# jolars/sgdnet

Measured on AMD Instinct MI355X. Metric: saga_epochs_per_sec, higher is better.
Workload: dtype f64

## Files before the change

sgdnet_amd/csrc/batched_k1.hpp:

```cpp
#pragma once

#include "batched_device.hpp"
#include "r_rng_word.hpp"

namespace sgdnet {


constexpr int kLanes8 = 8;

struct RecHeader {
  double y;
  int nnz;
  int ovf;
};

template <int kThreads>
__device__ __forceinline__ double k1_lanes8_draws(const SagaDev& d, const uint32_t* sp, int lo, int hi, double b0,
                                                  const double* wv, double* Dl) {
  typedef int ipair_t __attribute__((ext_vector_type(2)));
  typedef double dpair_t __attribute__((ext_vector_type(2)));
  constexpr int U = 4;
  constexpr int kG = kThreads / kLanes8;
  constexpr int kStep = kG * U;
  const int gl = threadIdx.x & (kLanes8 - 1);
// ... 65 lines not shown
          if (nz > kInReg8) {
            const int ov = __shfl(hd.ovf, 2 * u, kLanes8);
            row_for_each<kInReg8, kLanes8>(d, d.rec + (size_t)su[u] * stride, nz, ov, gl,
                      [&](int64_t j, double v) { scatter_add<true>(Dl + j, v * gc); });
          }
        }
      }
    }
    gct += gcp;
  }
  return gct;
}

constexpr int kCQ = 12;
constexpr int kCYOff = 112;
constexpr uint32_t kLongBit = 0x80000000u;
constexpr uint32_t kYBit = 0x20000000u;
constexpr int kCMOff = 120;

template <class F>
__device__ __forceinline__ void row_tail_compact(const SagaDev& d, uint32_t sid, int nnz, int gl, int E, F f) {
  const char* qb = d.cQ + (size_t)sid * kCStride;
  for (int e = E + 4 + gl; e < nnz; e += kLanes8) {
    if (e < E + kCQ) {
      f((int64_t) reinterpret_cast<const uint16_t*>(qb + 8)[e - E],
        reinterpret_cast<const double*>(qb + 32)[e - E]);
    } else {
      const int64_t q0 = d.ptr[sid];
      f((int64_t)d.idx[q0 + e], d.val[q0 + e]);
    }
  }
}

constexpr int kTicket = 32;

struct TicketSource {
  int* counter;
  int lo, hi, m;
  int t = 0;
  bool dynamic;
  __device__ __forceinline__ int next() {
    if (!dynamic) {
      const int b = lo + (t++ * (kLdsBlock / 64) + (int)(threadIdx.x >> 6)) * kTicket;
      return b < hi ? b : m;
    }
    int b = 0;
    if ((threadIdx.x & 63) == 0)
      b = __hip_atomic_fetch_add(counter, kTicket, __ATOMIC_RELAXED, __HIP_MEMORY_SCOPE_WORKGROUP);
    b = lo + __builtin_amdgcn_readfirstlane(b);
    return b < hi ? b : m;
  }
};

template <bool kRawStream>
struct K1CompactT {
  typedef double dpair_t __attribute__((ext_vector_type(2)));
  static constexpr int U = 4;
  int E, in_reg, gl, g, q, slot, id_off, v_off;
  bool y_in_meta, is_owner, in_p, half;
  const char* plane;
  char* P;
  const uint32_t* sp;
  const uint32_t* meta;
  int m;
  TicketSource tk;
  int b_cur, b_nxt;
  uint32_t s_cur, s_nxt;
  bool raw = false;
  const double* par = nullptr;

  __device__ __forceinline__ uint32_t sample_id(uint32_t x) const {
    if (kRawStream && raw) x = (uint32_t)par[1] + word_to_draw(x, par[0]);
    return x;
  }

  __device__ __forceinline__ int own_pos(int base) const { return base + U * g + q < m ? base + U * g + q : base; }
  __device__ __forceinline__ uint32_t tagged(uint32_t sid) const {
    const uint32_t mb = (meta[sid >> 4] >> (2 * (sid & 15))) & 3u;
    return sid | ((mb & 1u) ? kLongBit : 0u) | ((mb & 2u) ? kYBit : 0u);
  }
  static __device__ __forceinline__ int static_tickets() { return 2 * (kLdsBlock / 64) * kTicket; }

  __device__ __forceinline__ void init(const SagaDev& d, const uint32_t* sp_, int m_, int blk, int nblk,
                                       int* ticket_counter) {
    E = d.cE;
    in_reg = E + 4;
    y_in_meta = E == 12;
    gl = threadIdx.x & (kLanes8 - 1);
    g = (threadIdx.x & 63) >> 3;
    q = gl >> 1;
    is_owner = (gl & 1) == 0;
    in_p = gl < 6;
    slot = in_p ? gl : gl - 6;
    P = d.cP;
    plane = in_p ? d.cP : d.cQ;
    id_off = in_p ? 8 * E + 4 * slot : 8 + 4 * slot;
    v_off = in_p ? 16 * slot : 32 + 16 * slot;
    half = in_p && slot == 5 && E == 11;
    sp = sp_;
    meta = d.cmeta;
    m = m_;
    const int share = ((m + nblk - 1) / nblk + kTicket - 1) / kTicket * kTicket;
    tk.counter = ticket_counter;
    tk.lo = blk * share;
    tk.hi = tk.lo + share < m ? tk.lo + share : m;
    tk.m = m;
    tk.dynamic = share >= 4 * (kLdsBlock / 64) * kTicket;
    tk.t = 2;
    const int wave = (int)(threadIdx.x >> 6);
    b_cur = tk.lo + wave * kTicket;
    b_nxt = tk.lo + ((kLdsBlock / 64) + wave) * kTicket;
    if (b_cur >= tk.hi) b_cur = m;
    if (b_nxt >= tk.hi) b_nxt = m;
  }
  __device__ __forceinline__ void request_first() {
    s_cur = b_cur < m ? sp[own_pos(b_cur)] : 0u;
    s_nxt = b_nxt < m ? sp[own_pos(b_nxt)] : 0u;
  }
  __device__ __forceinline__ void begin(const SagaDev& d, const uint32_t* sp_, int m_, int blk, int nblk,
                                        int* ticket_counter) {
    init(d, sp_, m_, blk, nblk, ticket_counter);
    request_first();
  }

  __device__ __forceinline__ void tag_first() {
    if (b_cur < m) s_cur = tagged(sample_id(s_cur));
  }

  __device__ __forceinline__ double run(const SagaDev& d, double b0, const double* wv, double* Dl) {
    double gct = 0.0;
    while (b_cur < m) {
      const bool v_own = b_cur + U * g + q < m;
      uint32_t su[U];
#pragma unroll
      for (int u = 0; u < U; ++u) su[u] = (uint32_t)__shfl((int)s_cur, 2 * u, kLanes8);
      const uint32_t s_this = s_cur & kIdMask;
      double y_own = (s_cur & kYBit) ? 1.0 : 0.0;
      if (!y_in_meta) y_own = *reinterpret_cast<const double*>(P + (size_t)s_this * kCStride + kCYOff);
      int nnz_own = 0;
      if (s_cur & kLongBit) nnz_own = *reinterpret_cast<const int*>(d.cQ + (size_t)s_this * kCStride);
      uint32_t jf[U];
      dpair_t vf[U];
#pragma unroll
      for (int u = 0; u < U; ++u) {
        const bool on = in_p || (su[u] & kLongBit) != 0;
        const char* base = plane + (size_t)(su[u] & kIdMask) * kCStride;
        jf[u] = 0u;
        vf[u] = dpair_t{0.0, 0.0};
        if (on) {
          jf[u] = *reinterpret_cast<const uint32_t*>(base + id_off);
          vf[u] = *reinterpret_cast<const dpair_t*>(base + v_off);
        }
      }
      const int b_nn = b_nxt < m ? tk.next() : m;
      uint32_t s_nn = 0u;
      if (b_nn < m) s_nn = sp[own_pos(b_nn)];
      if (b_nxt < m) s_nxt = tagged(sample_id(s_nxt));
      if (half) {
#pragma unroll
        for (int u = 0; u < U; ++u) {
          vf[u].y = 0.0;
          jf[u] &= 0xffffu;
        }
      }
      double acc[U];
#pragma unroll
      for (int u = 0; u < U; ++u) acc[u] = vf[u].x * wv[jf[u] & 0xffffu] + vf[u].y * wv[jf[u] >> 16];
      const bool own_tail = v_own && nnz_own > in_reg;
      const bool any_tail = __ballot(own_tail) != 0;
      if (any_tail) {
#pragma unroll
        for (int u = 0; u < U; ++u) {
          const int nz = __shfl(own_tail ? nnz_own : 0, 2 * u, kLanes8);
          if (nz > in_reg) {
            double a = 0.0;
            row_tail_compact(d, su[u] & kIdMask, nz, gl, E, [&](int64_t j, double v) { a += v * wv[j]; });
            acc[u] += a;
          }
        }
      }
      const bool hi4 = (gl & 4) != 0, hi2 = (gl & 2) != 0;
      const double r0 = (hi4 ? acc[2] : acc[0]) + __shfl_xor(hi4 ? acc[0] : acc[2], 4, kLanes8);
      const double r1 = (hi4 ? acc[3] : acc[1]) + __shfl_xor(hi4 ? acc[1] : acc[3], 4, kLanes8);
      double t = (hi2 ? r1 : r0) + __shfl_xor(hi2 ? r0 : r1, 2, kLanes8);
      t += __shfl_xor(t, 1, kLanes8);
      const double lp = t + b0;
      const double g0 = d.family == SGDNET_BINOMIAL ? 1.0 - y_own - 1.0 / (1.0 + exp(lp)) : lp - y_own;
      double gcp = 0.0;
      if (is_owner && v_own) {
        const double old = __hip_atomic_exchange(reinterpret_cast<double*>(P + (size_t)s_this * kCStride + kCMOff), g0,
                                                 __ATOMIC_RELAXED, __HIP_MEMORY_SCOPE_AGENT);
        gcp = g0 - old;
      }
#pragma unroll
      for (int u = 0; u < U; ++u) {
        const double gc = __shfl(gcp, 2 * u, kLanes8);
        if (gc != 0.0) {
          if (vf[u].x != 0.0) scatter_add<true>(Dl + (jf[u] & 0xffffu), vf[u].x * gc);
          if (vf[u].y != 0.0) scatter_add<true>(Dl + (jf[u] >> 16), vf[u].y * gc);
          if (any_tail) {
            const int nz = __shfl(own_tail ? nnz_own : 0, 2 * u, kLanes8);
            if (nz > in_reg)
              row_tail_compact(d, su[u] & kIdMask, nz, gl, E,
                               [&](int64_t j, double v) { scatter_add<true>(Dl + j, v * gc); });
          }
        }
      }
      gct += gcp;
      s_cur = s_nxt;
      s_nxt = s_nn;
      b_cur = b_nxt;
      b_nxt = b_nn;
    }
    return gct;
  }
};
typedef K1CompactT<false> K1Compact;

template <int U>
struct K1IdsOnly {
  uint32_t s[U];
  bool valid[U];
  uint32_t s_own;
  bool v_own;
  bool valid_any;
  __device__ __forceinline__ void load(const SagaDev& d, const uint32_t* sp, int i, int hi, int step, int gl,
                                       int safe) {
#pragma unroll
    for (int u = 0; u < U; ++u) {
      const int iu = i + u * step;
      valid[u] = iu < hi;
      s[u] = sp[valid[u] ? iu : safe];
    }
    const int q = U == 4 ? gl >> 2 : gl;
    const int iq = i + q * step;
    v_own = q < U && iq < hi;
    s_own = sp[v_own ? iq : safe];
  }
};

template <int U>
struct K1Draws {
  uint32_t s[U];
  int jf[U], nnz[U];
  double vf[U];
  double gcp;
  bool valid[U];
  uint32_t s_own;
  double y_own;
  bool v_own;
  static __device__ __forceinline__ int draw_of(int gl) { return U == 4 ? gl >> 2 : gl; }

  static __device__ __forceinline__ int owner(int u) { return U == 4 ? 4 * u : u; }
  static __device__ __forceinline__ bool is_owner(int gl) { return U == 4 ? (gl & 3) == 0 : gl < U; }

  __device__ __forceinline__ void load_ids(const SagaDev& d, const uint32_t* sp, int i, int hi, int step, int gl,
// ... 112 lines not shown
```

sgdnet_amd/csrc/batched_shards.hip:

```cpp
#include "batched_k1.hpp"
#include "r_rng_bodies.hpp"

namespace sgdnet {

template <int KMAX>
__global__ __launch_bounds__(kBlock) void saga_vs_sweep_kernel(SagaDev d, LamParams* lamp, int tail, int nfb) {
  __shared__ double part[kSlabGroups][kSlabElems];
  __shared__ double red[kBlock / 64];
  __shared__ double sh_d0[KMAX];
  const SweepParams q = load_sweep_params(d, lamp, tail, SweepOverride{0.0, 0.0, 0.0});
  const int K = KMAX == 1 ? 1 : d.K;
  const int F = kSlabElems / K;
  const int E = F * K;
  const int v = (int)blockIdx.x / nfb, fb = (int)blockIdx.x - v * nfb;
  const int64_t KP = (int64_t)K * d.p;
  const double n_d = d.v_size[v];
  const int e = threadIdx.x % kSlabElems, g = threadIdx.x / kSlabElems;
  const int64_t elem = (int64_t)fb * E + e;
  const int64_t j_own = (int64_t)fb * F + threadIdx.x;
  const bool updates = (int)threadIdx.x < F && j_own < d.p;
  double w_old[KMAX], g_old[KMAX], c_own = 0.0;
#pragma unroll
  for (int k = 0; k < KMAX; ++k) {
    w_old[k] = g_old[k] = 0.0;
// ... 199 lines not shown
        return false;
      }
    }
  }
}

__device__ __forceinline__ bool fused_start(unsigned* sync, LamParams* lamp, unsigned grid) {
  unsigned* go = sync + kSyncGo * kSyncLine;
  const long long t0 = wall_clock64();
  if (blockIdx.x == 0) {
    unsigned expect = 0u;
    for (;;) {
      if (sync_load(sync, kSyncStart) >= grid) {
        __hip_atomic_compare_exchange_strong(go, &expect, 1u, __ATOMIC_RELAXED, __ATOMIC_RELAXED, __HIP_MEMORY_SCOPE_AGENT);
        break;
      }
      if (sync_load(sync, kSyncGo) != 0u) break;
      if (wall_clock64() - t0 > kFusedStartTicks) {
        __hip_atomic_compare_exchange_strong(go, &expect, 2u, __ATOMIC_RELAXED, __ATOMIC_RELAXED, __HIP_MEMORY_SCOPE_AGENT);
        break;
      }
      __builtin_amdgcn_s_sleep(4);
    }
  } else {
    for (;;) {
      if (sync_load(sync, kSyncGo) != 0u) break;
      if (wall_clock64() - t0 > 2 * kFusedStartTicks) {
        unsigned expect = 0u;
        __hip_atomic_compare_exchange_strong(go, &expect, 2u, __ATOMIC_RELAXED, __ATOMIC_RELAXED, __HIP_MEMORY_SCOPE_AGENT);
        break;
      }
      __builtin_amdgcn_s_sleep(4);
    }
  }
  const unsigned decision = sync_load(sync, kSyncGo);
  if (decision != 1u && decision != 3u) {
    __hip_atomic_store(&lamp->fused_abort, 1, __ATOMIC_RELAXED, __HIP_MEMORY_SCOPE_AGENT);
    __hip_atomic_fetch_max(sync + kSyncSticky * kSyncLine, 1u, __ATOMIC_RELAXED, __HIP_MEMORY_SCOPE_AGENT);
  }
  return decision == 1u;
}

__device__ __forceinline__ double fused_block_sum(double a, double* red) {
  a = wave_sum(a);
  if ((threadIdx.x & 63) == 0) red[threadIdx.x >> 6] = a;
  __syncthreads();
  double t = 0.0;
#pragma unroll
  for (int wv = 0; wv < kLdsBlock / 64; ++wv) t += red[wv];
  __syncthreads();
  return t;
}

__device__ __forceinline__ void fused_leave(const SagaDev& d, LamParams* lamp, int nb, bool epoch_done) {
  asm volatile("s_waitcnt vmcnt(0)" ::: "memory");
  __syncthreads();
  if (threadIdx.x == 0) {
    unsigned* sync = d.vsync;
    if (epoch_done && blockIdx.x == 0) {
      end_epoch(lamp, nb);
      if (d.n_peers > 1) __hip_atomic_fetch_add(sync + kSyncSeq * kSyncLine, 1u, __ATOMIC_RELAXED, __HIP_MEMORY_SCOPE_AGENT);
    }
    const unsigned prev = __hip_atomic_fetch_add(sync + kSyncExit * kSyncLine, 1u, __ATOMIC_RELAXED, __HIP_MEMORY_SCOPE_AGENT);
    if (prev + 1u == gridDim.x) {
      for (int wd = 0; wd < kSyncLines; ++wd)
        __hip_atomic_store(sync + wd * kSyncLine, 0u, __ATOMIC_RELAXED, __HIP_MEMORY_SCOPE_AGENT);
      if (!(d.n_peers > 1))
        for (int wd = 0; wd < kFusedMaxBps; ++wd)
          __hip_atomic_store(d.vcol + wd * kSyncLine, 0u, __ATOMIC_RELAXED, __HIP_MEMORY_SCOPE_AGENT);
      if (d.rngdev && lamp->rng_generate) d.rngdev->gen += 1u;
    }
  }
}

template <bool kPeers>
__global__ __launch_bounds__(kLdsBlock) void saga_vs_epoch_kernel(SagaDev d, LamParams* lamp, int nb, int every) {
  extern __shared__ __attribute__((aligned(16))) double Dl[];
  __shared__ int ticket_counter;
  __shared__ int sh_ok;
  __shared__ double sh_red[kLdsBlock / 64];
  __shared__ double sh_val[4];
  const int tid = threadIdx.x;
  const int64_t p = d.p;
  const int64_t P2 = p >> 1;
  const int S = d.v_bps, V = d.V;
  if ((int)blockIdx.x >= V * S) {
    if (d.rngdev && lamp->rng_generate) {
      const RngDev* R = d.rngdev;
      const unsigned gen = R->gen;
      uint32_t* lds = reinterpret_cast<uint32_t*>(Dl);
      const int rb = (int)blockIdx.x - V * S, nrb = (int)gridDim.x - V * S;
      mt_state_body(rb, nrb, reinterpret_cast<uint32_t(*)[2][kMtN + 1]>(lds), R->state[gen & 1u], R->ends,
                    R->stream + (int64_t)(gen & 1u) * R->n, R->n, R->seg, R->gens);
      __syncthreads();
      mt_jump_body(rb, nrb, lds, R->state[gen & 1u], R->state[(gen + 1u) & 1u], R->poly, R->gens);
    }
    fused_leave(d, lamp, nb, false);
    return;
  }
  const int v = (int)blockIdx.x % V, wi = (int)blockIdx.x / V;
  const int F = 2 * (int)((p + 2 * S - 1) / (2 * S));
  const int j0 = wi * F;
  const int jn = p - j0 < F ? (p - j0 > 0 ? (int)(p - j0) : 0) : F;
  double* Wl = Dl + p;
  f64x2_t* D2 = reinterpret_cast<f64x2_t*>(Dl);
  f64x2_t* W2 = reinterpret_cast<f64x2_t*>(Wl);
  const int penalty = lamp->penalty;
  __shared__ double sh_par[10];
  if (tid == 0) {
    sh_par[0] = lamp->gamma;
    sh_par[1] = lamp->beta;
    sh_par[2] = lamp->r_full;
    sh_par[3] = lamp->ls_full;
    sh_par[4] = lamp->r_tail;
    sh_par[5] = lamp->ls_tail;
    double tot = 0.0, lo = 0.0;
    for (int u = 0; u < d.V; ++u) {
      tot += d.v_size[u];
      if (u < (int)blockIdx.x % d.V) lo += d.v_size[u];
    }
    sh_par[6] = d.v_size[(int)blockIdx.x % d.V];
    sh_par[7] = lo;
    sh_par[8] = tot;
  }
  const int64_t m_full = lamp->m_full;
  const int64_t sbase = lamp->stream_base;
  const bool raw_words = lamp->stream_raw != 0;
  const int64_t dps = d.v_dps;
  const bool std_x = d.standardize != 0;
  const int64_t L = 2 * p + 2;
  double* vwv = d.vw + (int64_t)v * p;
  double* vGv = d.vG + (int64_t)v * p;
  double* refv = d.vx + (int64_t)v * L;
  double* cwp = d.vx + (int64_t)V * L;
  unsigned* sync = d.vsync;
  const __amdgpu_buffer_rsrc_t rs_slab = fused_rsrc(d.slab, (int64_t)V * S * p * 8);
  const __amdgpu_buffer_rsrc_t rs_w = fused_rsrc(vwv, p * 8);
  const uint32_t* const stream_v = d.stream + sbase + (int64_t)v * dps;
  typedef K1CompactT<true> K1Epoch;
  const double* const draw_par = sh_par + 6;

#ifdef SGDNET_PHASE_TIMING
  unsigned long long ph_t = 0;
  if (d.dbg && tid == 0) d.dbg[(size_t)blockIdx.x * 16 + 14] = ph_t = phase_stamp();
#define FPH(slot)                                                 \
  do {                                                            \
    if (d.dbg && tid == 0) {                                      \
      const unsigned long long now = phase_stamp();               \
      d.dbg[(size_t)blockIdx.x * 16 + (slot)] += now - ph_t;      \
      d.dbg[(size_t)blockIdx.x * 16 + 15] = ph_t = now;           \
    }                                                             \
  } while (0)
#else
#define FPH(slot) ((void)0)
#endif
  if (tid == 0) {
    const unsigned xcc = __builtin_amdgcn_s_getreg((3 << 11) | 20) & 15u;
    __hip_atomic_fetch_or(sync + (kSyncXcd + v) * kSyncLine, 1u << xcc, __ATOMIC_RELAXED, __HIP_MEMORY_SCOPE_AGENT);
    asm volatile("s_waitcnt vmcnt(0)" ::: "memory");
    __hip_atomic_fetch_add(sync + kSyncStart * kSyncLine, 1u, __ATOMIC_RELAXED, __HIP_MEMORY_SCOPE_AGENT);
    sh_ok = fused_start(sync, lamp, (unsigned)(V * S)) ? 1 : 0;
    if (sh_ok) {
      const unsigned mask = sync_load(sync, kSyncXcd + v);
      sh_ok = (mask & (mask - 1u)) == 0u ? 3 : 1;
    }
  }
  for (int64_t i = tid; i < P2; i += kLdsBlock) D2[i] = f64x2_t{0.0, 0.0};
  __syncthreads();
  bool done = false;
  bool alive = sh_ok != 0;
  unsigned col_base = 0u;
  if (kPeers) {
    int merges = 0;
    for (int r = 0; r < nb; ++r) merges += (r + 1 == nb || (r + 1) % every == 0) ? 1 : 0;
    col_base = sync_load(sync, kSyncSeq) * (unsigned)merges;
  }
  const bool local = (sh_ok & 2) != 0 && d.vs_xcd_local != 0;
  int mi = 0;
  uint32_t s_first = 0u, s_second = 0u;
  if (alive) {
    const int m0 = (int)(dps < m_full ? dps : m_full);
    K1Epoch nx;
    nx.begin(d, stream_v, m0, wi, S, &ticket_counter);
    s_first = nx.s_cur;
    s_second = nx.s_nxt;
  }
  for (int r = 0; alive && r < nb; ++r) {
    const int64_t t0 = (int64_t)r * m_full;
    const int m = (int)(dps - t0 < m_full ? dps - t0 : m_full);
    const bool tail = m != m_full;
    const bool last = r + 1 == nb;
    const bool merge_due = last || (r + 1) % every == 0;

    if (tid == 0) ticket_counter = K1Epoch::static_tickets();
    K1Epoch cg;
    cg.init(d, stream_v + t0, m, wi, S, &ticket_counter);
    cg.raw = raw_words;
    cg.par = draw_par;
    cg.s_cur = s_first;
    cg.s_nxt = s_second;
    cg.tag_first();
    int ts = threadIdx.x;
    asm volatile("" : "+v"(ts));
    double cw = 0.0, bv = 0.0;
    if ((ts >> 6) == 0) {
      if (std_x && r > 0)
        for (int k = ts & 63; k < S; k += 64) cw += ld_sc1(cwp + v * kFusedMaxBps + k);
      bv = r == 0 ? d.b[0] : ld_sc1(d.vb + v);
    }
    {
      constexpr int kStage = 8;
      for (int64_t i0 = ts; i0 < P2; i0 += (int64_t)kLdsBlock * kStage) {
        f64x2_t t[kStage];
#pragma unroll
        for (int q = 0; q < kStage; ++q) {
          const int64_t i = i0 + (int64_t)q * kLdsBlock;
          t[q] = f64x2_t{0.0, 0.0};
          if (i < P2) t[q] = r == 0 ? reinterpret_cast<const f64x2_t*>(d.w)[i] : ld2_sc1(rs_w, (uint32_t)(i * 16));
        }
#pragma unroll
        for (int q = 0; q < kStage; ++q) {
          const int64_t i = i0 + (int64_t)q * kLdsBlock;
          if (i < P2) W2[i] = t[q];
        }
      }
    }
    if ((ts >> 6) == 0) {
      cw = wave_sum(cw);
      if ((ts & 63) == 0) sh_val[0] = bv - cw;
    }
    __syncthreads();
    if (r == 0 && std_x) {
      double a = 0.0;
      for (int64_t j = ts; j < p; j += kLdsBlock) a += d.c[j] * Wl[j];
      a = fused_block_sum(a, sh_red);
      if (ts == 0) sh_val[0] -= a;
      __syncthreads();
    }
    const double b0 = sh_val[0];
    FPH(0);

    const double gct = cg.run(d, b0, Wl, Dl);
    __syncthreads();
    FPH(1);
    int tq = threadIdx.x;
    asm volatile("" : "+v"(tq));
    const int lane = tq & 63, wave = tq >> 6;
    const int64_t t0n = t0 + m_full;
    const int mn = (int)(dps - t0n < m_full ? dps - t0n : m_full);

    {
      const uint32_t base = (uint32_t)(((int64_t)blockIdx.x * p) * 8);
      for (int64_t i = tq; i < P2; i += kLdsBlock) {
        st2_shard(D2[i], rs_slab, base + (uint32_t)(i * 16), local);
        D2[i] = f64x2_t{0.0, 0.0};
      }
      const double t = wave_sum(gct);
      if (lane == 0) sh_red[wave] = t;
      __syncthreads();
      if (tq == 0) {
        double tot = 0.0;
        for (int wv = 0; wv < kLdsBlock / 64; ++wv) tot += sh_red[wv];
        st_shard(d.vd0 + blockIdx.x, tot, local);
      }
    }
    fused_arrive(sync, kSyncCnt1 + v);
    FPH(2);
    const bool upd = tq < jn;
    const bool icpt = wi == 0 && tq == jn;
    const bool act = upd || icpt;
    const int64_t j = j0 + tq;
    const int64_t oa = upd ? j : 2 * p, ob = upd ? p + j : 2 * p + 1;
    double* const rep_a = upd ? vGv + j : d.vgb + v;
    double* const rep_b = upd ? vwv + j : d.vb + v;
    const double* const own_a = upd ? d.G + j : d.gb;
    const double* const own_b = upd ? d.w + j : d.b;
    double a_old = 0.0, b_old = 0.0, c_own = 0.0, ra = 0.0, rb = 0.0;
    if (act) {
      a_old = r == 0 ? *own_a : ld_sc1(rep_a);
      b_old = r == 0 ? *own_b : ld_sc1(rep_b);
      if (std_x && upd) c_own = d.c[j];
      if (merge_due) {
        ra = mi == 0 ? *own_a : ld_sc1(refv + oa);
        rb = mi == 0 ? *own_b : ld_sc1(refv + ob);
      }
    }
    if (tq == 0) sh_ok = fused_poll(sync, kSyncCnt1 + v, (unsigned)S * (unsigned)(r + 1), lamp) ? 1 : 0;
    __syncthreads();
    if (!sh_ok) break;
    FPH(3);

    {
      double gsum = 0.0;
      if (wave == kLdsBlock / 64 - 1)
        for (int k = lane; k < S; k += 64) gsum += ld_sc1(d.vd0 + k * V + v);
      f64x2_t acc[kFusedChunks];
#pragma unroll
      for (int c = 0; c < kFusedChunks; ++c) acc[c] = f64x2_t{0.0, 0.0};
      for (int k = wave; k < S; k += 2 * (kLdsBlock / 64)) {
        const bool two = k + kLdsBlock / 64 < S;
        const uint32_t o0 = (uint32_t)((((int64_t)(k * V + v)) * p + j0) * 8);
        const uint32_t o1 = (uint32_t)((((int64_t)((k + kLdsBlock / 64) * V + v)) * p + j0) * 8);
        f64x2_t a0[kFusedChunks], a1[kFusedChunks];
#pragma unroll
        for (int c = 0; c < kFusedChunks; ++c) {
          const int pi = c * 64 + lane;
          a0[c] = a1[c] = f64x2_t{0.0, 0.0};
          if (2 * pi < jn) {
            a0[c] = ld2_sc1(rs_slab, o0 + (uint32_t)(pi * 16));
            if (two) a1[c] = ld2_sc1(rs_slab, o1 + (uint32_t)(pi * 16));
          }
        }
#pragma unroll
        for (int c = 0; c < kFusedChunks; ++c) {
          acc[c] += a0[c];
          acc[c] += a1[c];
        }
      }
#pragma unroll
      for (int c = 0; c < kFusedChunks; ++c) {
        const int pi = c * 64 + lane;
        if (2 * pi < F) reinterpret_cast<f64x2_t*>(Wl + (int64_t)wave * F)[pi] = acc[c];
      }
      if (wave == kLdsBlock / 64 - 1) {
        gsum = wave_sum(gsum);
        if (lane == 0) sh_val[1] = gsum;
      }
    }
    __syncthreads();
    double a_new = a_old, b_new = b_old;
    {
      const double d0 = sh_val[1];
      const double n_d = sh_par[6], gamma = sh_par[0];
      if (upd) {
        double dj = 0.0;
#pragma unroll
        for (int wv = 0; wv < kLdsBlock / 64; ++wv) dj += Wl[(int64_t)wv * F + tq];
        if (std_x) dj -= c_own * d0;
        const double beta = sh_par[1];
        const double r_m = tail ? sh_par[4] : sh_par[2], ls_m = tail ? sh_par[5] : sh_par[3];
        const double val = r_m * b_old - (gamma * ls_m) * a_old - gamma * dj;
        const double tau = beta * gamma * ls_m;
        b_new = val;
        if (penalty == SGDNET_ELASTICNET) {
          b_new = soft_threshold(val, tau);
        } else if (penalty == SGDNET_GROUPLASSO) {
          const double factor = tau / sqrt(val * val);
          b_new = factor < 1.0 ? val * (1.0 - factor) : 0.0;
        }
        a_new = (dj != 0.0 || penalty == SGDNET_GROUPLASSO) ? a_old + dj / n_d : a_old;
      } else if (icpt && d.fit_intercept) {
        const double dk = d0 / n_d;
        a_new = a_old + dk;
        b_new = b_old - gamma * (a_new * (d.xd ? 1.0 : 0.01) * (double)m + dk);
      }
    }
    FPH(4);
    if (merge_due) {
      const FusedPeers* PR = kPeers ? d.peers : nullptr;
      const int NP = kPeers ? d.n_peers : 1;
      double* pubv = d.vpub + (int64_t)((mi & 1) * V + v) * L;
      if (PR) {
        if (act) {
          st_sys(pubv + oa, a_new);
          st_sys(pubv + ob, b_new);
        }
        asm volatile("s_waitcnt vmcnt(0)" ::: "memory");
        __syncthreads();
        if (tq == 0)
          for (int q = 0; q < NP; ++q)
            __hip_atomic_fetch_add(PR->sync[q] + wi * kSyncLine, 1u, __ATOMIC_RELAXED, __HIP_MEMORY_SCOPE_SYSTEM);
      } else {
        if (act) {
          st_sc1(pubv + oa, a_new);
          st_sc1(pubv + ob, b_new);
        }
        fused_arrive(d.vcol, wi);
      }
      if (tq == 0)
        sh_ok = fused_poll(d.vcol, wi, (unsigned)(NP * V) * (col_base + (unsigned)(mi + 1)), lamp, PR != nullptr, sync) ? 1 : 0;
      __syncthreads();
      if (!sh_ok) break;
      double ma = ra, mb = rb;
      const double tot_all = PR ? PR->tot_size : sh_par[8];
      for (int q = 0; q < NP; ++q) {
        const double* pub0 = (PR ? PR->pub[q] : d.vpub) + (int64_t)((mi & 1) * V) * L;
        double xa[8], xb[8];
#pragma unroll
        for (int u = 0; u < 8; ++u) {
          xa[u] = xb[u] = 0.0;
          if (u < V && act) {
            xa[u] = PR ? ld_sys(pub0 + (int64_t)u * L + oa) : ld_sc1(pub0 + (int64_t)u * L + oa);
            xb[u] = PR ? ld_sys(pub0 + (int64_t)u * L + ob) : ld_sc1(pub0 + (int64_t)u * L + ob);
          }
        }
#pragma unroll
        for (int u = 0; u < 8; ++u) {
          if (u < V) {
            const double wt = (PR ? PR->vsize[q][u] : d.v_size[u]) / tot_all;
            ma += wt * (xa[u] - ra);
            mb += wt * (xb[u] - rb);
          }
        }
      }
      if (act) {
        a_new = ma;
        b_new = mb;
        st_sc1(refv + oa, ma);
        st_sc1(refv + ob, mb);
        if (last && v == 0) {
          *const_cast<double*>(own_a) = ma;
          *const_cast<double*>(own_b) = mb;
        }
      }
      ++mi;
      FPH(5);
    }
    if (act) {
      st_shard(rep_a, a_new, local);
      st_shard(rep_b, b_new, local);
    }
    if (std_x) {
      const double a = fused_block_sum(upd ? c_own * b_new : 0.0, sh_red);
      if (tq == 0) st_shard(cwp + v * kFusedMaxBps + wi, a, local);
    }
    if (last) {
      done = true;
      break;
    }
    fused_arrive(sync, kSyncCnt2 + v);
    FPH(6);
    {
      K1Epoch nx;
      nx.begin(d, stream_v + t0n, mn, wi, S, &ticket_counter);
      s_first = nx.s_cur;
      s_second = nx.s_nxt;
    }
    if (tq == 0) sh_ok = fused_poll(sync, kSyncCnt2 + v, (unsigned)S * (unsigned)(r + 1), lamp) ? 1 : 0;
    __syncthreads();
    if (!sh_ok) break;
    FPH(7);
  }

  fused_leave(d, lamp, nb, done);
}

int launch_vs_broadcast(const SagaDev& d, hipStream_t st) {
  const int64_t len = 2 * (int64_t)d.K * d.p + 2 * d.K;
  return launch_kernel(saga_vs_broadcast_kernel, dim3(clamped_grid(len, kBlock, 1024)), dim3(kBlock), 0, 0, st, nullptr,
                       nullptr, d);
}

int launch_vs_cw(const SagaDev& d, hipStream_t st) {
  if (!d.standardize) return SGDNET_OK;
  return launch_kernel(saga_vs_cw_kernel, dim3(d.V * d.K), dim3(kBlock), 0, 0, st, nullptr, nullptr, d);
}

int launch_vs_merge(const SagaDev& d, int final_merge, hipStream_t st, LamParams* epoch_end, int batches) {
  const int64_t len = 2 * (int64_t)d.K * d.p + 2 * d.K;
  return launch_kernel(saga_vs_merge_kernel, dim3(clamped_grid(len, kBlock, 1024)), dim3(kBlock), 0, 0, st, nullptr,
                       nullptr, d, final_merge, epoch_end, batches);
}

int launch_vs_sweep(const SagaDev& d, const BatchPlan& g, LamParams* lam, int tail, hipStream_t st, hipEvent_t ev0,
                    hipEvent_t ev1) {
  const int F = kSlabElems / d.K;
  const int nfb = (int)((d.p + F - 1) / F);
  return with_class_width(g.kw, [&](auto kw) {
    return launch_kernel(saga_vs_sweep_kernel<decltype(kw)::value>, dim3(nfb * d.V), dim3(kBlock), 0, 0, st, ev0, ev1, d,
                         lam, tail, nfb);
  });
}

int launch_vs_epoch(const SagaDev& d, const BatchPlan& g, LamParams* lam, int nb, int every, hipStream_t st,
                    hipEvent_t ev0, hipEvent_t ev1) {
  if (nb < 1 || every < 1) return SGDNET_EINVAL;
  const bool peers = d.n_peers > 1 && d.peers;
  return launch_kernel(peers ? saga_vs_epoch_kernel<true> : saga_vs_epoch_kernel<false>, dim3(g.grid), dim3(kLdsBlock),
                       g.lds_bytes, kLdsAll, st, ev0, ev1, d, lam, nb, every);
}

}
```

Before: 1252.

## Specialize fused epoch kernel on record width and family; reload args from kernarg

Makes the per-record entry count and the loss family template parameters of the compact sampler and the fused epoch kernel, so lane offsets, the half-slot mask and the gradient formula become compile-time constants. The fused kernel also stops holding many SagaDev-derived values live across the epoch loop. It rereads them from the kernarg segment through a pointer and readfirstlane, and stashes lamp scalars in shared memory. The aim is lower register pressure and less scalar work in the hot loop. Combinations not covered (for example E=12 with Gaussian) now return an unsupported error.

```diff
diff --git a/sgdnet_amd/csrc/batched_k1.hpp b/sgdnet_amd/csrc/batched_k1.hpp
--- a/sgdnet_amd/csrc/batched_k1.hpp
+++ b/sgdnet_amd/csrc/batched_k1.hpp
@@ -141,12 +141,22 @@
   }
 };
 
-template <bool kRawStream>
+constexpr int kGeomRunTime = 0;
+constexpr int kFamilyRunTime = -1;
+template <bool kRawStream, int kE = kGeomRunTime, int kFamily = kFamilyRunTime>
 struct K1CompactT {
+  static_assert(kE == kGeomRunTime || kE == 11 || kE == 12, "plane P holds 11 or 12 entries");
   typedef double dpair_t __attribute__((ext_vector_type(2)));
   static constexpr int U = 4;
-  int E, in_reg, gl, g, q, slot, id_off, v_off;
-  bool y_in_meta, is_owner, in_p, half;
+  int E_rt, gl, g, q, slot, id_off, v_off;
+  bool y_in_meta_rt, is_owner, in_p, half_rt;
+  __device__ __forceinline__ int entries() const { return kE == kGeomRunTime ? E_rt : kE; }
+  __device__ __forceinline__ int in_reg() const { return entries() + 4; }
+  __device__ __forceinline__ bool y_in_meta() const { return kE == kGeomRunTime ? y_in_meta_rt : kE == 12; }
+  __device__ __forceinline__ bool half() const { return kE == kGeomRunTime ? half_rt : kE == 11 && in_p && slot == 5; }
+  __device__ __forceinline__ bool binomial(const SagaDev& d) const {
+    return kFamily == kFamilyRunTime ? d.family == SGDNET_BINOMIAL : kFamily == SGDNET_BINOMIAL;
+  }
   const char* plane;
   char* P;
   const uint32_t* sp;
@@ -172,9 +182,10 @@
 
   __device__ __forceinline__ void init(const SagaDev& d, const uint32_t* sp_, int m_, int blk, int nblk,
                                        int* ticket_counter) {
-    E = d.cE;
-    in_reg = E + 4;
-    y_in_meta = E == 12;
+    if (kE == kGeomRunTime) {
+      E_rt = d.cE;
+      y_in_meta_rt = E_rt == 12;
+    }
     gl = threadIdx.x & (kLanes8 - 1);
     g = (threadIdx.x & 63) >> 3;
     q = gl >> 1;
@@ -183,9 +194,9 @@
     slot = in_p ? gl : gl - 6;
     P = d.cP;
     plane = in_p ? d.cP : d.cQ;
-    id_off = in_p ? 8 * E + 4 * slot : 8 + 4 * slot;
+    id_off = in_p ? 8 * entries() + 4 * slot : 8 + 4 * slot;
     v_off = in_p ? 16 * slot : 32 + 16 * slot;
-    half = in_p && slot == 5 && E == 11;
+    if (kE == kGeomRunTime) half_rt = in_p && slot == 5 && E_rt == 11;
     sp = sp_;
     meta = d.cmeta;
     m = m_;
@@ -225,7 +236,7 @@
       for (int u = 0; u < U; ++u) su[u] = (uint32_t)__shfl((int)s_cur, 2 * u, kLanes8);
       const uint32_t s_this = s_cur & kIdMask;
       double y_own = (s_cur & kYBit) ? 1.0 : 0.0;
-      if (!y_in_meta) y_own = *reinterpret_cast<const double*>(P + (size_t)s_this * kCStride + kCYOff);
+      if (!y_in_meta()) y_own = *reinterpret_cast<const double*>(P + (size_t)s_this * kCStride + kCYOff);
       int nnz_own = 0;
       if (s_cur & kLongBit) nnz_own = *reinterpret_cast<const int*>(d.cQ + (size_t)s_this * kCStride);
       uint32_t jf[U];
@@ -245,7 +256,7 @@
       uint32_t s_nn = 0u;
       if (b_nn < m) s_nn = sp[own_pos(b_nn)];
       if (b_nxt < m) s_nxt = tagged(sample_id(s_nxt));
-      if (half) {
+      if (half()) {
 #pragma unroll
         for (int u = 0; u < U; ++u) {
           vf[u].y = 0.0;
@@ -255,15 +266,15 @@
       double acc[U];
 #pragma unroll
       for (int u = 0; u < U; ++u) acc[u] = vf[u].x * wv[jf[u] & 0xffffu] + vf[u].y * wv[jf[u] >> 16];
-      const bool own_tail = v_own && nnz_own > in_reg;
+      const bool own_tail = v_own && nnz_own > in_reg();
       const bool any_tail = __ballot(own_tail) != 0;
       if (any_tail) {
 #pragma unroll
         for (int u = 0; u < U; ++u) {
           const int nz = __shfl(own_tail ? nnz_own : 0, 2 * u, kLanes8);
-          if (nz > in_reg) {
+          if (nz > in_reg()) {
             double a = 0.0;
-            row_tail_compact(d, su[u] & kIdMask, nz, gl, E, [&](int64_t j, double v) { a += v * wv[j]; });
+            row_tail_compact(d, su[u] & kIdMask, nz, gl, entries(), [&](int64_t j, double v) { a += v * wv[j]; });
             acc[u] += a;
           }
         }
@@ -274,7 +285,7 @@
       double t = (hi2 ? r1 : r0) + __shfl_xor(hi2 ? r0 : r1, 2, kLanes8);
       t += __shfl_xor(t, 1, kLanes8);
       const double lp = t + b0;
-      const double g0 = d.family == SGDNET_BINOMIAL ? 1.0 - y_own - 1.0 / (1.0 + exp(lp)) : lp - y_own;
+      const double g0 = binomial(d) ? 1.0 - y_own - 1.0 / (1.0 + exp(lp)) : lp - y_own;
       double gcp = 0.0;
       if (is_owner && v_own) {
         const double old = __hip_atomic_exchange(reinterpret_cast<double*>(P + (size_t)s_this * kCStride + kCMOff), g0,
@@ -289,8 +300,8 @@
           if (vf[u].y != 0.0) scatter_add<true>(Dl + (jf[u] >> 16), vf[u].y * gc);
           if (any_tail) {
             const int nz = __shfl(own_tail ? nnz_own : 0, 2 * u, kLanes8);
-            if (nz > in_reg)
-              row_tail_compact(d, su[u] & kIdMask, nz, gl, E,
+            if (nz > in_reg())
+              row_tail_compact(d, su[u] & kIdMask, nz, gl, entries(),
                                [&](int64_t j, double v) { scatter_add<true>(Dl + j, v * gc); });
           }
         }
diff --git a/sgdnet_amd/csrc/batched_shards.hip b/sgdnet_amd/csrc/batched_shards.hip
--- a/sgdnet_amd/csrc/batched_shards.hip
+++ b/sgdnet_amd/csrc/batched_shards.hip
@@ -275,13 +275,46 @@
   return t;
 }
 
-__device__ __forceinline__ void fused_leave(const SagaDev& d, LamParams* lamp, int nb, bool epoch_done) {
+struct FusedArgs {
+  SagaDev d;
+  LamParams* lamp;
+  int nb, every;
+};
+static_assert(offsetof(FusedArgs, lamp) == sizeof(SagaDev) && offsetof(FusedArgs, every) == sizeof(SagaDev) + 12,
+              "the kernarg segment of saga_vs_epoch_kernel(SagaDev, LamParams*, int, int)");
+typedef const FusedArgs __attribute__((address_space(4))) * FusedArgsPtr;
+__device__ __forceinline__ FusedArgsPtr fused_args() {
+  FusedArgsPtr a = (FusedArgsPtr)__builtin_amdgcn_kernarg_segment_ptr();
+  asm volatile("" : "+s"(a));
+  return a;
+}
+__device__ __forceinline__ int64_t fused_uniform(long long x) {
+  const uint32_t lo = (uint32_t)__builtin_amdgcn_readfirstlane((int)x);
+  const uint32_t hi = (uint32_t)__builtin_amdgcn_readfirstlane((int)(x >> 32));
+  return (int64_t)(((unsigned long long)hi << 32) | lo);
+}
+struct FusedWho {
+  int V, S, v, wi;
+};
+__device__ __forceinline__ FusedWho fused_who(FusedArgsPtr a) {
+  FusedWho g;
+  g.V = a->d.V;
+  g.S = a->d.v_bps;
+  g.v = (int)blockIdx.x % g.V;
+  g.wi = (int)blockIdx.x / g.V;
+  return g;
+}
+
+__device__ __forceinline__ void fused_leave(bool epoch_done) {
   asm volatile("s_waitcnt vmcnt(0)" ::: "memory");
   __syncthreads();
   if (threadIdx.x == 0) {
+    const FusedArgsPtr a = fused_args();
+    const auto& d = a->d;
+    LamParams* lamp = a->lamp;
     unsigned* sync = d.vsync;
     if (epoch_done && blockIdx.x == 0) {
-      end_epoch(lamp, nb);
+      end_epoch(lamp, a->nb);
       if (d.n_peers > 1) __hip_atomic_fetch_add(sync + kSyncSeq * kSyncLine, 1u, __ATOMIC_RELAXED, __HIP_MEMORY_SCOPE_AGENT);
     }
     const unsigned prev = __hip_atomic_fetch_add(sync + kSyncExit * kSyncLine, 1u, __ATOMIC_RELAXED, __HIP_MEMORY_SCOPE_AGENT);
@@ -296,178 +329,217 @@
   }
 }
 
-template <bool kPeers>
-__global__ __launch_bounds__(kLdsBlock) void saga_vs_epoch_kernel(SagaDev d, LamParams* lamp, int nb, int every) {
+template <bool kPeers, int kE, int kFamily>
+__global__ __launch_bounds__(kLdsBlock) void saga_vs_epoch_kernel(SagaDev d, LamParams*, int, int) {
   extern __shared__ __attribute__((aligned(16))) double Dl[];
   __shared__ int ticket_counter;
   __shared__ int sh_ok;
   __shared__ double sh_red[kLdsBlock / 64];
   __shared__ double sh_val[4];
+  __shared__ double sh_par[10];
+  __shared__ long long sh_lam[4];
   const int tid = threadIdx.x;
-  const int64_t p = d.p;
-  const int64_t P2 = p >> 1;
-  const int S = d.v_bps, V = d.V;
-  if ((int)blockIdx.x >= V * S) {
-    if (d.rngdev && lamp->rng_generate) {
-      const RngDev* R = d.rngdev;
-      const unsigned gen = R->gen;
-      uint32_t* lds = reinterpret_cast<uint32_t*>(Dl);
-      const int rb = (int)blockIdx.x - V * S, nrb = (int)gridDim.x - V * S;
-      mt_state_body(rb, nrb, reinterpret_cast<uint32_t(*)[2][kMtN + 1]>(lds), R->state[gen & 1u], R->ends,
-                    R->stream + (int64_t)(gen & 1u) * R->n, R->n, R->seg, R->gens);
-      __syncthreads();
-      mt_jump_body(rb, nrb, lds, R->state[gen & 1u], R->state[(gen + 1u) & 1u], R->poly, R->gens);
-    }
-    fused_leave(d, lamp, nb, false);
-    return;
-  }
-  const int v = (int)blockIdx.x % V, wi = (int)blockIdx.x / V;
-  const int F = 2 * (int)((p + 2 * S - 1) / (2 * S));
-  const int j0 = wi * F;
-  const int jn = p - j0 < F ? (p - j0 > 0 ? (int)(p - j0) : 0) : F;
-  double* Wl = Dl + p;
+  {
+    const FusedArgsPtr a = fused_args();
+    const int V = a->d.V, S = a->d.v_bps;
+    if ((int)blockIdx.x >= V * S) {
+      if (a->d.rngdev && a->lamp->rng_generate) {
+        const RngDev* R = a->d.rngdev;
+        const unsigned gen = R->gen;
+        uint32_t* lds = reinterpret_cast<uint32_t*>(Dl);
+        const int rb = (int)blockIdx.x - V * S, nrb = (int)gridDim.x - V * S;
+        mt_state_body(rb, nrb, reinterpret_cast<uint32_t(*)[2][kMtN + 1]>(lds), R->state[gen & 1u], R->ends,
+                      R->stream + (int64_t)(gen & 1u) * R->n, R->n, R->seg, R->gens);
+        __syncthreads();
+        mt_jump_body(rb, nrb, lds, R->state[gen & 1u], R->state[(gen + 1u) & 1u], R->poly, R->gens);
+      }
+      fused_leave(false);
+      return;
+    }
+  }
   f64x2_t* D2 = reinterpret_cast<f64x2_t*>(Dl);
-  f64x2_t* W2 = reinterpret_cast<f64x2_t*>(Wl);
-  const int penalty = lamp->penalty;
-  __shared__ double sh_par[10];
-  if (tid == 0) {
-    sh_par[0] = lamp->gamma;
-    sh_par[1] = lamp->beta;
-    sh_par[2] = lamp->r_full;
-    sh_par[3] = lamp->ls_full;
-    sh_par[4] = lamp->r_tail;
-    sh_par[5] = lamp->ls_tail;
-    double tot = 0.0, lo = 0.0;
-    for (int u = 0; u < d.V; ++u) {
-      tot += d.v_size[u];
-      if (u < (int)blockIdx.x % d.V) lo += d.v_size[u];
-    }
-    sh_par[6] = d.v_size[(int)blockIdx.x % d.V];
-    sh_par[7] = lo;
-    sh_par[8] = tot;
-  }
-  const int64_t m_full = lamp->m_full;
-  const int64_t sbase = lamp->stream_base;
-  const bool raw_words = lamp->stream_raw != 0;
-  const int64_t dps = d.v_dps;
-  const bool std_x = d.standardize != 0;
-  const int64_t L = 2 * p + 2;
-  double* vwv = d.vw + (int64_t)v * p;
-  double* vGv = d.vG + (int64_t)v * p;
-  double* refv = d.vx + (int64_t)v * L;
-  double* cwp = d.vx + (int64_t)V * L;
-  unsigned* sync = d.vsync;
-  const __amdgpu_buffer_rsrc_t rs_slab = fused_rsrc(d.slab, (int64_t)V * S * p * 8);
-  const __amdgpu_buffer_rsrc_t rs_w = fused_rsrc(vwv, p * 8);
-  const uint32_t* const stream_v = d.stream + sbase + (int64_t)v * dps;
-  typedef K1CompactT<true> K1Epoch;
   const double* const draw_par = sh_par + 6;
 
 #ifdef SGDNET_PHASE_TIMING
   unsigned long long ph_t = 0;
-  if (d.dbg && tid == 0) d.dbg[(size_t)blockIdx.x * 16 + 14] = ph_t = phase_stamp();
+  if (tid == 0) {
+    unsigned long long* dbg = fused_args()->d.dbg;
+    if (dbg) dbg[(size_t)blockIdx.x * 16 + 14] = ph_t = phase_stamp();
+  }
 #define FPH(slot)                                                 \
   do {                                                            \
-    if (d.dbg && tid == 0) {                                      \
-      const unsigned long long now = phase_stamp();               \
-      d.dbg[(size_t)blockIdx.x * 16 + (slot)] += now - ph_t;      \
-      d.dbg[(size_t)blockIdx.x * 16 + 15] = ph_t = now;           \
+    if (tid == 0) {                                               \
+      unsigned long long* dbg = fused_args()->d.dbg;              \
+      if (dbg) {                                                  \
+        const unsigned long long now = phase_stamp();             \
+        dbg[(size_t)blockIdx.x * 16 + (slot)] += now - ph_t;      \
+        dbg[(size_t)blockIdx.x * 16 + 15] = ph_t = now;           \
+      }                                                           \
     }                                                             \
   } while (0)
 #else
 #define FPH(slot) ((void)0)
 #endif
-  if (tid == 0) {
-    const unsigned xcc = __builtin_amdgcn_s_getreg((3 << 11) | 20) & 15u;
-    __hip_atomic_fetch_or(sync + (kSyncXcd + v) * kSyncLine, 1u << xcc, __ATOMIC_RELAXED, __HIP_MEMORY_SCOPE_AGENT);
-    asm volatile("s_waitcnt vmcnt(0)" ::: "memory");
-    __hip_atomic_fetch_add(sync + kSyncStart * kSyncLine, 1u, __ATOMIC_RELAXED, __HIP_MEMORY_SCOPE_AGENT);
-    sh_ok = fused_start(sync, lamp, (unsigned)(V * S)) ? 1 : 0;
-    if (sh_ok) {
-      const unsigned mask = sync_load(sync, kSyncXcd + v);
-      sh_ok = (mask & (mask - 1u)) == 0u ? 3 : 1;
-    }
-  }
-  for (int64_t i = tid; i < P2; i += kLdsBlock) D2[i] = f64x2_t{0.0, 0.0};
-  __syncthreads();
   bool done = false;
-  bool alive = sh_ok != 0;
+  bool alive;
+  bool local;
   unsigned col_base = 0u;
-  if (kPeers) {
-    int merges = 0;
-    for (int r = 0; r < nb; ++r) merges += (r + 1 == nb || (r + 1) % every == 0) ? 1 : 0;
-    col_base = sync_load(sync, kSyncSeq) * (unsigned)merges;
-  }
-  const bool local = (sh_ok & 2) != 0 && d.vs_xcd_local != 0;
+  uint32_t s_first = 0u, s_second = 0u;
+  {
+    const FusedArgsPtr a = fused_args();
+    const FusedWho g = fused_who(a);
+    LamParams* lamp = a->lamp;
+    unsigned* sync = a->d.vsync;
+    if (tid == 0) {
+      sh_par[0] = lamp->gamma;
+      sh_par[1] = lamp->beta;
+      sh_par[2] = lamp->r_full;
+      sh_par[3] = lamp->ls_full;
+      sh_par[4] = lamp->r_tail;
+      sh_par[5] = lamp->ls_tail;
+      double tot = 0.0, lo = 0.0;
+      for (int u = 0; u < g.V; ++u) {
+        tot += a->d.v_size[u];
+        if (u < g.v) lo += a->d.v_size[u];
+      }
+      sh_par[6] = a->d.v_size[g.v];
+      sh_par[7] = lo;
+      sh_par[8] = tot;
+      sh_lam[0] = lamp->m_full;
+      sh_lam[1] = lamp->stream_base;
+      sh_lam[2] = lamp->penalty;
+      sh_lam[3] = lamp->stream_raw;
+      const unsigned xcc = __builtin_amdgcn_s_getreg((3 << 11) | 20) & 15u;
+      __hip_atomic_fetch_or(sync + (kSyncXcd + g.v) * kSyncLine, 1u << xcc, __ATOMIC_RELAXED, __HIP_MEMORY_SCOPE_AGENT);
+      asm volatile("s_waitcnt vmcnt(0)" ::: "memory");
+      __hip_atomic_fetch_add(sync + kSyncStart * kSyncLine, 1u, __ATOMIC_RELAXED, __HIP_MEMORY_SCOPE_AGENT);
+      sh_ok = fused_start(sync, lamp, (unsigned)(g.V * g.S)) ? 1 : 0;
+      if (sh_ok) {
+        const unsigned mask = sync_load(sync, kSyncXcd + g.v);
+        sh_ok = (mask & (mask - 1u)) == 0u ? 3 : 1;
+      }
+    }
+    const int64_t P2 = a->d.p >> 1;
+    for (int64_t i = tid; i < P2; i += kLdsBlock) D2[i] = f64x2_t{0.0, 0.0};
+    __syncthreads();
+    const int ok = __builtin_amdgcn_readfirstlane(sh_ok);
+    alive = ok != 0;
+    if (kPeers) {
+      const int nb = a->nb, every = a->every;
+      int merges = 0;
+      for (int r = 0; r < nb; ++r) merges += (r + 1 == nb || (r + 1) % every == 0) ? 1 : 0;
+      col_base = sync_load(sync, kSyncSeq) * (unsigned)merges;
+    }
+    local = (ok & 2) != 0 && a->d.vs_xcd_local != 0;
+    if (alive) {
+      const int64_t m_full = fused_uniform(sh_lam[0]), dps = a->d.v_dps;
+      const int m0 = (int)(dps < m_full ? dps : m_full);
+      const uint32_t* stream_v = a->d.stream + fused_uniform(sh_lam[1]) + (int64_t)g.v * dps;
+      K1CompactT<true, kE, kFamily> nx;
+      nx.begin(d, stream_v, m0, g.wi, g.S, &ticket_counter);
+      s_first = nx.s_cur;
+      s_second = nx.s_nxt;
+    }
+  }
+  typedef K1CompactT<true, kE, kFamily> K1Epoch;
   int mi = 0;
-  uint32_t s_first = 0u, s_second = 0u;
-  if (alive) {
-    const int m0 = (int)(dps < m_full ? dps : m_full);
-    K1Epoch nx;
-    nx.begin(d, stream_v, m0, wi, S, &ticket_counter);
-    s_first = nx.s_cur;
-    s_second = nx.s_nxt;
-  }
-  for (int r = 0; alive && r < nb; ++r) {
-    const int64_t t0 = (int64_t)r * m_full;
-    const int m = (int)(dps - t0 < m_full ? dps - t0 : m_full);
-    const bool tail = m != m_full;
-    const bool last = r + 1 == nb;
-    const bool merge_due = last || (r + 1) % every == 0;
-
-    if (tid == 0) ticket_counter = K1Epoch::static_tickets();
-    K1Epoch cg;
-    cg.init(d, stream_v + t0, m, wi, S, &ticket_counter);
-    cg.raw = raw_words;
-    cg.par = draw_par;
-    cg.s_cur = s_first;
-    cg.s_nxt = s_second;
-    cg.tag_first();
-    int ts = threadIdx.x;
-    asm volatile("" : "+v"(ts));
-    double cw = 0.0, bv = 0.0;
-    if ((ts >> 6) == 0) {
-      if (std_x && r > 0)
-        for (int k = ts & 63; k < S; k += 64) cw += ld_sc1(cwp + v * kFusedMaxBps + k);
-      bv = r == 0 ? d.b[0] : ld_sc1(d.vb + v);
-    }
+  for (int r = 0; alive && r < fused_args()->nb; ++r) {
+    double gct, *Wl;
     {
-      constexpr int kStage = 8;
-      for (int64_t i0 = ts; i0 < P2; i0 += (int64_t)kLdsBlock * kStage) {
-        f64x2_t t[kStage];
-#pragma unroll
-        for (int q = 0; q < kStage; ++q) {
-          const int64_t i = i0 + (int64_t)q * kLdsBlock;
-          t[q] = f64x2_t{0.0, 0.0};
-          if (i < P2) t[q] = r == 0 ? reinterpret_cast<const f64x2_t*>(d.w)[i] : ld2_sc1(rs_w, (uint32_t)(i * 16));
-        }
-#pragma unroll
-        for (int q = 0; q < kStage; ++q) {
-          const int64_t i = i0 + (int64_t)q * kLdsBlock;
-          if (i < P2) W2[i] = t[q];
-        }
-      }
-    }
-    if ((ts >> 6) == 0) {
-      cw = wave_sum(cw);
-      if ((ts & 63) == 0) sh_val[0] = bv - cw;
-    }
-    __syncthreads();
-    if (r == 0 && std_x) {
-      double a = 0.0;
-      for (int64_t j = ts; j < p; j += kLdsBlock) a += d.c[j] * Wl[j];
-      a = fused_block_sum(a, sh_red);
-      if (ts == 0) sh_val[0] -= a;
+      const FusedArgsPtr a = fused_args();
+      const FusedWho g = fused_who(a);
+      const int64_t p = a->d.p, P2 = p >> 1;
+      const int64_t m_full = fused_uniform(sh_lam[0]), dps = a->d.v_dps;
+      const int64_t t0 = (int64_t)r * m_full;
+      const int m = (int)(dps - t0 < m_full ? dps - t0 : m_full);
+      const uint32_t* stream_v = a->d.stream + fused_uniform(sh_lam[1]) + (int64_t)g.v * dps;
+      const bool std_x = a->d.standardize != 0;
+      Wl = Dl + p;
+      f64x2_t* W2 = reinterpret_cast<f64x2_t*>(Wl);
+      if (tid == 0) ticket_counter = K1Epoch::static_tickets();
+      K1Epoch cg;
+      cg.init(d, stream_v + t0, m, g.wi, g.S, &ticket_counter);
+      cg.raw = __builtin_amdgcn_readfirstlane((int)sh_lam[3]) != 0;
+      cg.par = draw_par;
+      cg.s_cur = s_first;
+      cg.s_nxt = s_second;
+      cg.tag_first();
+      int ts = threadIdx.x;
+      asm volatile("" : "+v"(ts));
+      double cw = 0.0, bv = 0.0;
+      if ((ts >> 6) == 0) {
+        if (std_x && r > 0) {
+          const double* cwp = a->d.vx + (int64_t)g.V * (2 * p + 2);
+          for (int k = ts & 63; k < g.S; k += 64) cw += ld_sc1(cwp + g.v * kFusedMaxBps + k);
+        }
+        bv = r == 0 ? a->d.b[0] : ld_sc1(a->d.vb + g.v);
+      }
+      {
+        constexpr int kStage = 8;
+        const __amdgpu_buffer_rsrc_t rs_w = fused_rsrc(a->d.vw + (int64_t)g.v * p, p * 8);
+        const f64x2_t* w2 = reinterpret_cast<const f64x2_t*>(a->d.w);
+        for (int64_t i0 = ts; i0 < P2; i0 += (int64_t)kLdsBlock * kStage) {
+          f64x2_t t[kStage];
+#pragma unroll
+          for (int q = 0; q < kStage; ++q) {
+            const int64_t i = i0 + (int64_t)q * kLdsBlock;
+            t[q] = f64x2_t{0.0, 0.0};
+            if (i < P2) t[q] = r == 0 ? w2[i] : ld2_sc1(rs_w, (uint32_t)(i * 16));
+          }
+#pragma unroll
+          for (int q = 0; q < kStage; ++q) {
+            const int64_t i = i0 + (int64_t)q * kLdsBlock;
+            if (i < P2) W2[i] = t[q];
+          }
+        }
+      }
+      if ((ts >> 6) == 0) {
+        cw = wave_sum(cw);
+        if ((ts & 63) == 0) sh_val[0] = bv - cw;
+      }
       __syncthreads();
-    }
-    const double b0 = sh_val[0];
-    FPH(0);
-
-    const double gct = cg.run(d, b0, Wl, Dl);
+      if (r == 0 && std_x) {
+        const double* c = a->d.c;
+        double s = 0.0;
+        for (int64_t j = ts; j < p; j += kLdsBlock) s += c[j] * Wl[j];
+        s = fused_block_sum(s, sh_red);
+        if (ts == 0) sh_val[0] -= s;
+        __syncthreads();
+      }
+      const double b0 = sh_val[0];
+      FPH(0);
+
+      gct = cg.run(d, b0, Wl, Dl);
+    }
     __syncthreads();
     FPH(1);
     int tq = threadIdx.x;
     asm volatile("" : "+v"(tq));
+    const FusedArgsPtr a = fused_args();
+    const auto& da = a->d;
+    const FusedWho g = fused_who(a);
+    const int S = g.S, V = g.V, v = g.v, wi = g.wi;
+    const int64_t p = da.p, P2 = p >> 1;
+    const int F = 2 * (int)((p + 2 * S - 1) / (2 * S));
+    const int j0 = wi * F;
+    const int jn = p - j0 < F ? (p - j0 > 0 ? (int)(p - j0) : 0) : F;
+    const int64_t m_full = fused_uniform(sh_lam[0]), dps = da.v_dps;
+    const int64_t t0 = (int64_t)r * m_full;
+    const int m = (int)(dps - t0 < m_full ? dps - t0 : m_full);
+    const bool tail = m != m_full;
+    const int nb = a->nb;
+    const bool last = r + 1 == nb;
+    const bool merge_due = last || (r + 1) % a->every == 0;
+    const int penalty = __builtin_amdgcn_readfirstlane((int)sh_lam[2]);
+    const bool std_x = da.standardize != 0;
+    const int64_t L = 2 * p + 2;
+    LamParams* lamp = a->lamp;
+    double* vwv = da.vw + (int64_t)v * p;
+    double* vGv = da.vG + (int64_t)v * p;
+    double* refv = da.vx + (int64_t)v * L;
+    double* cwp = da.vx + (int64_t)V * L;
+    unsigned* sync = da.vsync;
+    const __amdgpu_buffer_rsrc_t rs_slab = fused_rsrc(da.slab, (int64_t)V * S * p * 8);
     const int lane = tq & 63, wave = tq >> 6;
     const int64_t t0n = t0 + m_full;
     const int mn = (int)(dps - t0n < m_full ? dps - t0n : m_full);
@@ -484,7 +556,7 @@
       if (tq == 0) {
         double tot = 0.0;
         for (int wv = 0; wv < kLdsBlock / 64; ++wv) tot += sh_red[wv];
-        st_shard(d.vd0 + blockIdx.x, tot, local);
+        st_shard(da.vd0 + blockIdx.x, tot, local);
       }
     }
     fused_arrive(sync, kSyncCnt1 + v);
@@ -494,15 +566,15 @@
     const bool act = upd || icpt;
     const int64_t j = j0 + tq;
     const int64_t oa = upd ? j : 2 * p, ob = upd ? p + j : 2 * p + 1;
-    double* const rep_a = upd ? vGv + j : d.vgb + v;
-    double* const rep_b = upd ? vwv + j : d.vb + v;
-    const double* const own_a = upd ? d.G + j : d.gb;
-    const double* const own_b = upd ? d.w + j : d.b;
+    double* const rep_a = upd ? vGv + j : da.vgb + v;
+    double* const rep_b = upd ? vwv + j : da.vb + v;
+    const double* const own_a = upd ? da.G + j : da.gb;
+    const double* const own_b = upd ? da.w + j : da.b;
     double a_old = 0.0, b_old = 0.0, c_own = 0.0, ra = 0.0, rb = 0.0;
     if (act) {
       a_old = r == 0 ? *own_a : ld_sc1(rep_a);
       b_old = r == 0 ? *own_b : ld_sc1(rep_b);
-      if (std_x && upd) c_own = d.c[j];
+      if (std_x && upd) c_own = da.c[j];
       if (merge_due) {
         ra = mi == 0 ? *own_a : ld_sc1(refv + oa);
         rb = mi == 0 ? *own_b : ld_sc1(refv + ob);
@@ -516,7 +588,7 @@
     {
       double gsum = 0.0;
       if (wave == kLdsBlock / 64 - 1)
-        for (int k = lane; k < S; k += 64) gsum += ld_sc1(d.vd0 + k * V + v);
+        for (int k = lane; k < S; k += 64) gsum += ld_sc1(da.vd0 + k * V + v);
       f64x2_t acc[kFusedChunks];
 #pragma unroll
       for (int c = 0; c < kFusedChunks; ++c) acc[c] = f64x2_t{0.0, 0.0};
@@ -572,17 +644,17 @@
           b_new = factor < 1.0 ? val * (1.0 - factor) : 0.0;
         }
         a_new = (dj != 0.0 || penalty == SGDNET_GROUPLASSO) ? a_old + dj / n_d : a_old;
-      } else if (icpt && d.fit_intercept) {
+      } else if (icpt && da.fit_intercept) {
         const double dk = d0 / n_d;
         a_new = a_old + dk;
-        b_new = b_old - gamma * (a_new * (d.xd ? 1.0 : 0.01) * (double)m + dk);
+        b_new = b_old - gamma * (a_new * (da.xd ? 1.0 : 0.01) * (double)m + dk);
       }
     }
     FPH(4);
     if (merge_due) {
-      const FusedPeers* PR = kPeers ? d.peers : nullptr;
-      const int NP = kPeers ? d.n_peers : 1;
-      double* pubv = d.vpub + (int64_t)((mi & 1) * V + v) * L;
+      const FusedPeers* PR = kPeers ? da.peers : nullptr;
+      const int NP = kPeers ? da.n_peers : 1;
+      double* pubv = da.vpub + (int64_t)((mi & 1) * V + v) * L;
       if (PR) {
         if (act) {
           st_sys(pubv + oa, a_new);
@@ -598,16 +670,16 @@
           st_sc1(pubv + oa, a_new);
           st_sc1(pubv + ob, b_new);
         }
-        fused_arrive(d.vcol, wi);
+        fused_arrive(da.vcol, wi);
       }
       if (tq == 0)
-        sh_ok = fused_poll(d.vcol, wi, (unsigned)(NP * V) * (col_base + (unsigned)(mi + 1)), lamp, PR != nullptr, sync) ? 1 : 0;
+        sh_ok = fused_poll(da.vcol, wi, (unsigned)(NP * V) * (col_base + (unsigned)(mi + 1)), lamp, PR != nullptr, sync) ? 1 : 0;
       __syncthreads();
       if (!sh_ok) break;
       double ma = ra, mb = rb;
       const double tot_all = PR ? PR->tot_size : sh_par[8];
       for (int q = 0; q < NP; ++q) {
-        const double* pub0 = (PR ? PR->pub[q] : d.vpub) + (int64_t)((mi & 1) * V) * L;
+        const double* pub0 = (PR ? PR->pub[q] : da.vpub) + (int64_t)((mi & 1) * V) * L;
         double xa[8], xb[8];
 #pragma unroll
         for (int u = 0; u < 8; ++u) {
@@ -620,7 +692,7 @@
 #pragma unroll
         for (int u = 0; u < 8; ++u) {
           if (u < V) {
-            const double wt = (PR ? PR->vsize[q][u] : d.v_size[u]) / tot_all;
+            const double wt = (PR ? PR->vsize[q][u] : da.v_size[u]) / tot_all;
             ma += wt * (xa[u] - ra);
             mb += wt * (xb[u] - rb);
           }
@@ -644,8 +716,8 @@
       st_shard(rep_b, b_new, local);
     }
     if (std_x) {
-      const double a = fused_block_sum(upd ? c_own * b_new : 0.0, sh_red);
-      if (tq == 0) st_shard(cwp + v * kFusedMaxBps + wi, a, local);
+      const double s = fused_block_sum(upd ? c_own * b_new : 0.0, sh_red);
+      if (tq == 0) st_shard(cwp + v * kFusedMaxBps + wi, s, local);
     }
     if (last) {
       done = true;
@@ -654,6 +726,7 @@
     fused_arrive(sync, kSyncCnt2 + v);
     FPH(6);
     {
+      const uint32_t* stream_v = da.stream + fused_uniform(sh_lam[1]) + (int64_t)v * dps;
       K1Epoch nx;
       nx.begin(d, stream_v + t0n, mn, wi, S, &ticket_counter);
       s_first = nx.s_cur;
@@ -665,7 +738,7 @@
     FPH(7);
   }
 
-  fused_leave(d, lamp, nb, done);
+  fused_leave(done);
 }
 
 int launch_vs_broadcast(const SagaDev& d, hipStream_t st) {
@@ -699,8 +772,19 @@
                     hipEvent_t ev0, hipEvent_t ev1) {
   if (nb < 1 || every < 1) return SGDNET_EINVAL;
   const bool peers = d.n_peers > 1 && d.peers;
-  return launch_kernel(peers ? saga_vs_epoch_kernel<true> : saga_vs_epoch_kernel<false>, dim3(g.grid), dim3(kLdsBlock),
-                       g.lds_bytes, kLdsAll, st, ev0, ev1, d, lam, nb, every);
-}
-
-}
+  const bool binomial = d.family == SGDNET_BINOMIAL;
+  void (*kernel)(SagaDev, LamParams*, int, int) = nullptr;
+  if (d.cE == 12 && binomial)
+    kernel = peers ? saga_vs_epoch_kernel<true, 12, SGDNET_BINOMIAL> : saga_vs_epoch_kernel<false, 12, SGDNET_BINOMIAL>;
+  else if (d.cE == 11 && !binomial)
+    kernel = peers ? saga_vs_epoch_kernel<true, 11, SGDNET_GAUSSIAN> : saga_vs_epoch_kernel<false, 11, SGDNET_GAUSSIAN>;
+  else if (d.cE == 11 && binomial)
+    kernel = peers ? saga_vs_epoch_kernel<true, 11, SGDNET_BINOMIAL> : saga_vs_epoch_kernel<false, 11, SGDNET_BINOMIAL>;
+  if (!kernel) {
+    set_error("fused epoch: no kernel for %d entries per record and family %d", d.cE, d.family);
+    return SGDNET_EUNSUPPORTED;
+  }
+  return launch_kernel(kernel, dim3(g.grid), dim3(kLdsBlock), g.lds_bytes, kLdsAll, st, ev0, ev1, d, lam, nb, every);
+}
+
+}
```

Result: faster. 1306, median of 6 (+4.3%).
